# timmh/biolith

Hardware: AMD Instinct MI355X
Metric: effective samples/sec (psi) for occu NUTS, 10k sites x 5 visits (higher is better)
Workload: dtype f32; 1 GPU; biolith simulate(n_sites=10000, n_site_covs=3, n_obs_covs=3, 5 visits, seed 0); fit(occu): NUTS 4 chains per GPU x (1000 warmup + 1000 draws), one step = one full fit; chains_per_gpu=4, total_chains=4, num_warmup=1000, num_samples=1000, parallelism=chains x1 (1 process per GPU), wgs_per_chain=27, gather=none (one rank), env_overrides=

## Files before the change

### biolith_amd/csrc/biolith_hip.hip

```cpp
#include "../../include/biolith_hip.h"

#include <hip/hip_runtime.h>

#include <algorithm>
#include <cmath>
#include <cstdarg>
#include <cstdio>
#include <cstdlib>
#include <cstring>
#include <string>
#include <vector>

#include "logp_kernel.hpp"
#include "re_kernel.hpp"
#include "nuts_kernel.hpp"
#include "predict.hpp"
#include "site_posterior.hpp"
#include "abundance_posterior.hpp"
#include "path_posterior.hpp"
#include "score_posterior.hpp"
#include "count_posterior.hpp"
#include "comb_predict.hpp"
#include "predictive_check.hpp"
#include "predictive_density.hpp"
// ... 1700 lines not shown
        if (const char *e = bl_env(BL_ENV_RE_WGS)) k = atoi(e);
    }
    int ncu = 256;
    { hipDeviceProp_t prop; if (hipGetDeviceProperties(&prop, ds->device) == hipSuccess && prop.multiProcessorCount > 0) ncu = prop.multiProcessorCount; }
    k = std::max(1, std::min(std::min(k, 32), std::min(ncu * 7 / 8 / C, N * g.n_species)));
    const int nsp = g.n_species;
    int kps = std::max(1, k / nsp);
    const int nloc = (N + kps - 1) / kps;
    kps = (N + nloc - 1) / nloc;
    k = nsp * kps;
    if (k > 32) return bl_fail(BL_ERR_UNSUPPORTED, "n_species=%d needs %d workgroups per chain (at most 32)", nsp, k);
    if (C * k > ncu) return bl_fail(BL_ERR_UNSUPPORTED, "num_chains=%d random-effects chains need %d resident workgroups (%d CUs)", C, C * k, ncu);
    const int dl_max = g.G + nloc * per_site;

    const RunLayout RL = result_layout((size_t)C, Sa, D);
    size_t off = RL.end;
    auto carve = [&](size_t bytes) { size_t o = off; off = align256(off + bytes); return o; };
    const size_t o_draws = RL.draws, o_div = RL.div, o_steps = RL.steps, o_acc = RL.acc, o_pot = RL.pot, o_eps = RL.eps,
                 o_minv = RL.minv, o_nleap = RL.nleap, o_status = carve(16),
                 o_rng = carve((size_t)C * k * (dl_max + 2) * 16), o_init = carve((size_t)C * D * 4), o_dbg = carve(BL_DBG_SLOTS * 8),
                 o_xchg = carve((size_t)C * 2 * k * BL_RE_NRED_MAX * 8), o_loc = carve((size_t)C * 4), o_run = carve(sizeof(BlReRun));
    if (off > ds->run_bytes) {
        if (ds->d_run) hipFree(ds->d_run);
        ds->d_run = nullptr; ds->run_bytes = 0;
        BL_HIP(hipMalloc(&ds->d_run, off));
        ds->run_bytes = off;
    }
    const size_t state_bytes = (size_t)C * k * RE_SLOTS * dl_max * 4;
    if (state_bytes > ds->restate_bytes) {
        if (ds->d_restate) hipFree(ds->d_restate);
        ds->d_restate = nullptr; ds->restate_bytes = 0;
        BL_HIP(hipMalloc((void **)&ds->d_restate, state_bytes));
        ds->restate_bytes = state_bytes;
    }
    char *base = (char *)ds->d_run;
    ds->d_draws = (float *)(base + o_draws); ds->d_div = (unsigned char *)(base + o_div); ds->d_steps = (int *)(base + o_steps);
    ds->d_acc = (float *)(base + o_acc); ds->d_pot = (float *)(base + o_pot); ds->d_eps = (float *)(base + o_eps);
    ds->d_minv = (float *)(base + o_minv); ds->d_nleap = (long long *)(base + o_nleap); ds->d_status = (int *)(base + o_status);
    ds->d_rng = (uint32_t *)(base + o_rng); ds->d_init = (float *)(base + o_init); ds->d_dbg = (long long *)(base + o_dbg);
    ds->d_loc = (int *)(base + o_loc);

    const bool small_layout = D + 2 <= (size_t)BL_RNG_STREAMS_PER_CHAIN - 1;
    const int stride = small_layout ? BL_RNG_STREAMS_PER_CHAIN : (int)D + 2;
    const int ext_scalar = small_layout ? BL_RNG_STREAMS_PER_CHAIN - 1 : (int)D, ext_dir = small_layout ? BL_RNG_STREAMS_PER_CHAIN - 2 : (int)D + 1;
    std::vector<uint32_t> all((size_t)C * stride * 4), rs((size_t)C * k * (dl_max + 2) * 4, 0u);
    rng_streams_strided(cfg->seed, cfg->chain_offset, stride, C, all.data());
    for (int c = 0; c < C; c++)
        for (int w = 0; w < k; w++) {
            const int sp = w / kps, s0 = (w - sp * kps) * nloc, cnt = std::min(nloc, N - s0);
            uint32_t *dst = rs.data() + ((size_t)c * k + w) * (dl_max + 2) * 4;
            const uint32_t *src = all.data() + (size_t)c * stride * 4;
            auto put = [&](int local, int ext) { memcpy(dst + (size_t)local * 4, src + (size_t)ext * 4, 16); };
            int at = 0;
            for (; at < g.G; at++) put(at, at);
            if (g.site_re) {
                for (int i = 0; i < cnt; i++) put(at + i, g.o_u + sp * N + s0 + i);
                for (int i = 0; i < cnt; i++) put(at + cnt + i, g.o_v + sp * N + s0 + i);
                at += 2 * cnt;
            }
            if (g.obs_re)
                for (int v = 0; v < V; v++)
                    for (int i = 0; i < cnt; i++) put(at + v * cnt + i, g.o_e + (sp * N + s0 + i) * V + v);
            put(dl_max, ext_scalar);
            put(dl_max + 1, ext_dir);
        }
    BL_HIP(hipMemcpyAsync(ds->d_rng, rs.data(), rs.size() * 4, hipMemcpyHostToDevice, st));
    std::vector<float> it32;
    if (cfg->init_theta) {
        it32.resize((size_t)C * D);
        for (size_t i = 0; i < it32.size(); i++) it32[i] = (float)cfg->init_theta[i];
        BL_HIP(hipMemcpyAsync(ds->d_init, it32.data(), it32.size() * 4, hipMemcpyHostToDevice, st));
    }
    BlReRun run{};
    run.m = g;
    run.comb = ds->comb;
    const size_t lds = re_geometry(run.m, nloc, 1, dl_max);
    const bool cap4 = g.Ks <= 4 && g.Ko <= 4;
    run.num_chains = C; run.num_warmup = W; run.num_samples = S; run.max_depth = max_depth;
    run.k = k; run.nloc = nloc; run.dl_max = dl_max;
    run.xchg = (unsigned long long *)(base + o_xchg);
    { const char *e1 = bl_env(BL_ENV_NO_LOCAL); run.allow_local = (e1 && e1[0] == '1') ? 0 : 1; }
    run.xcd_local = ds->d_loc;
    run.target_accept = (float)(cfg->target_accept > 0.0 ? cfg->target_accept : 0.8);
    int32_t ws[32], we[32];
    run.nwin = adaptation_schedule(W, ws, we, 32);
    if (run.nwin > 32) return bl_fail(BL_ERR_INVALID, "adaptation schedule too long");
    for (int i = 0; i < 32; i++) run.win_end[i] = i < run.nwin ? we[i] : 0x7fffffff;
    run.state = ds->d_restate; run.rng = ds->d_rng;
    run.init_theta = cfg->init_theta ? ds->d_init : nullptr;
    run.abort_flag = ds->d_abort;
    run.draws = ds->d_draws; run.diverging = ds->d_div; run.num_steps = ds->d_steps; run.accept_prob = ds->d_acc;
    run.potential = ds->d_pot; run.step_size = ds->d_eps; run.inv_mass = ds->d_minv; run.nleap = ds->d_nleap; run.status = ds->d_status;
    run.dbg = ds->d_dbg;
    BlReRun *d_runp = (BlReRun *)(base + o_run);
    BL_HIP(hipMemcpyAsync(d_runp, &run, sizeof run, hipMemcpyHostToDevice, st));
    BL_HIP(hipStreamSynchronize(st));
    *ds->h_abort = 0;
    BL_HIP(hipEventRecord(ds->ev0, st));
    BL_HIP(hipMemsetAsync(ds->d_status, 0, 16, st));
    BL_HIP(hipMemsetAsync(ds->d_dbg, 0, BL_DBG_SLOTS * 8, st));
    BL_HIP(hipMemsetAsync(run.xchg, 0, (size_t)C * 2 * k * BL_RE_NRED_MAX * 8, st));
    BL_HIP(hipMemsetAsync(ds->d_loc, 0, (size_t)C * 4, st));
    BL_HIP(re_nuts_dispatch(cap4 ? 4 : 16, run, 8 * k * ((C + 7) / 8), lds, st));
    snprintf(ds->kernel_name, sizeof ds->kernel_name, "%s", g_kernel_name);
    BL_HIP(hipEventRecord(ds->ev1, st));
    ds->stream = st; ds->in_flight = true; ds->have_run = true;
    ds->C = C; ds->S = S; ds->W = W; ds->k = k; ds->nloc = nloc; ds->lds_ld = 0; ds->lds_bytes = (int)lds; ds->staged = run.m.lds_rows | (run.m.lds_hot << 1); ds->nvp = 0; ds->ncw = BL_RE_NW; ds->lane_grp = 0;
    return BL_OK;
}

extern "C" int bl_nuts_launch(bl_dataset *ds, const bl_nuts_config *cfg, void *stream)
{
    if (!ds || !cfg) return bl_fail(BL_ERR_INVALID, "NULL argument");
    if (ds->in_flight) return bl_fail(BL_ERR_BUSY, "a NUTS launch is already in flight on this handle");
    bl_env_snapshot();
    snprintf(ds->env_overrides, sizeof ds->env_overrides, "%s", bl_env_active().c_str());
    const int C = cfg->num_chains, S = cfg->num_samples, W = cfg->num_warmup, D = ds->D;
    if (C <= 0 || S < 0 || W < 0 || S + W <= 0) return bl_fail(BL_ERR_INVALID, "num_chains/num_samples/num_warmup out of range");
    if (C > 256) return bl_fail(BL_ERR_UNSUPPORTED, "num_chains=%d > 256 per device launch", C);
    const int max_depth = cfg->max_tree_depth > 0 ? cfg->max_tree_depth : 10;
    if (max_depth > BL_MAX_DEPTH) return bl_fail(BL_ERR_INVALID, "max_tree_depth > %d", BL_MAX_DEPTH);
    if (cfg->chain_offset < 0) return bl_fail(BL_ERR_INVALID, "chain_offset < 0");
    int rc = set_device(ds);
    if (rc) return rc;

    if (ds->model == 6) return re_nuts_launch(ds, cfg, (hipStream_t)stream, max_depth);

    int k, nloc, ld, lds_bytes, staged;
    int ncw, wide, grp;
    choose_geometry(ds, C, cfg->wgs_per_chain, &k, &nloc, &ld, &lds_bytes, &staged, &ncw, &wide, &grp);
    const int nvp = (D + 4 <= 16) ? 16 : (D + 4 <= 32 ? 32 : 64);

    const size_t Sa = S > 0 ? S : 1;
    const RunLayout RL = result_layout((size_t)C, Sa, (size_t)D);
    size_t off = RL.end;
    auto carve = [&](size_t bytes) { size_t o = off; off = align256(off + bytes); return o; };
    const size_t o_draws = RL.draws, o_div = RL.div, o_steps = RL.steps, o_acc = RL.acc, o_pot = RL.pot, o_eps = RL.eps,
                 o_minv = RL.minv, o_nleap = RL.nleap, o_status = carve(16),
                 o_rng = carve((size_t)C * BL_RNG_STREAMS_PER_CHAIN * 16), o_init = carve((size_t)C * D * 4), o_dbg = carve(BL_DBG_SLOTS * 8), o_loc = carve((size_t)C * 4),
                 o_cold = carve(sizeof(BlNutsCold));
    if (off > ds->run_bytes) {
        if (ds->d_run) hipFree(ds->d_run);
        ds->d_run = nullptr; ds->run_bytes = 0;
        BL_HIP(hipMalloc(&ds->d_run, off));
        ds->run_bytes = off;
    }
    char *base = (char *)ds->d_run;
    ds->d_draws = (float *)(base + o_draws); ds->d_div = (unsigned char *)(base + o_div); ds->d_steps = (int *)(base + o_steps);
    ds->d_acc = (float *)(base + o_acc); ds->d_pot = (float *)(base + o_pot); ds->d_eps = (float *)(base + o_eps);
    ds->d_minv = (float *)(base + o_minv); ds->d_nleap = (long long *)(base + o_nleap); ds->d_status = (int *)(base + o_status);
    ds->d_rng = (uint32_t *)(base + o_rng); ds->d_init = (float *)(base + o_init); ds->d_dbg = (long long *)(base + o_dbg); ds->d_loc = (int *)(base + o_loc);
    int pitch = nvp;
    { const char *e = bl_env(BL_ENV_PITCH); if (e && atoi(e) >= nvp && atoi(e) <= 4096) pitch = atoi(e); }
    const size_t xb = align256((size_t)C * BL_XCHG_SLOTS * k * pitch * 8);
    if (xb > ds->xchg_bytes) {
        if (ds->d_xchg) hipFree(ds->d_xchg);
        ds->d_xchg = nullptr; ds->xchg_bytes = 0;
        BL_HIP(hipMalloc((void **)&ds->d_xchg, xb));
        ds->xchg_bytes = xb;
    }

    hipStream_t st = (hipStream_t)stream;
    std::vector<uint32_t> rs((size_t)C * BL_RNG_STREAMS_PER_CHAIN * 4);
    for (int c = 0; c < C; c++)
        rng_streams(cfg->seed, cfg->chain_offset + c, BL_RNG_STREAMS_PER_CHAIN, rs.data() + (size_t)c * BL_RNG_STREAMS_PER_CHAIN * 4);
    BL_HIP(hipMemcpyAsync(ds->d_rng, rs.data(), rs.size() * 4, hipMemcpyHostToDevice, st));
    if (cfg->init_theta) {
        std::vector<float> it32((size_t)C * D);
        for (size_t i = 0; i < it32.size(); i++) it32[i] = (float)cfg->init_theta[i];
        BL_HIP(hipMemcpyAsync(ds->d_init, it32.data(), it32.size() * 4, hipMemcpyHostToDevice, st));
    }
    BlNutsCold cold{};
    cold.num_warmup = W; cold.num_samples = S;
    cold.target_accept = (float)(cfg->target_accept > 0.0 ? cfg->target_accept : 0.8);
    int32_t ws[32], we[32];
    cold.nwin = adaptation_schedule(W, ws, we, 32);
    if (cold.nwin > 32) return bl_fail(BL_ERR_INVALID, "adaptation schedule too long");
    for (int i = 0; i < 32; i++) cold.win_end[i] = i < cold.nwin ? we[i] : 0x7fffffff;
    cold.loc_b = ds->dd.loc_b; cold.isc2_b = ds->dd.isc2_b; cold.loc_a = ds->dd.loc_a; cold.isc2_a = ds->dd.isc2_a;
    cold.l1_b = ds->dd.l1_b; cold.l1_a = ds->dd.l1_a;
    cold.prior_const = ds->dd.prior_const;
    cold.fp_a = (float)ds->fp_a; cold.fp_b = (float)ds->fp_b;
    cold.rng = ds->d_rng;
    cold.init_theta = cfg->init_theta ? ds->d_init : nullptr;
    cold.abort_flag = ds->d_abort;
    cold.draws = ds->d_draws; cold.diverging = ds->d_div; cold.num_steps = ds->d_steps; cold.accept_prob = ds->d_acc;
    cold.potential = ds->d_pot; cold.step_size = ds->d_eps; cold.inv_mass = ds->d_minv; cold.nleap = ds->d_nleap;
    cold.status = ds->d_status; cold.xcd_local = ds->d_loc; cold.dbg = ds->d_dbg;
    BlNutsCold *d_cold = (BlNutsCold *)(base + o_cold);
    BL_HIP(hipMemcpyAsync(d_cold, &cold, sizeof cold, hipMemcpyHostToDevice, st));
    BL_HIP(hipStreamSynchronize(st));
    *ds->h_abort = 0;

    BlNutsParams p{};
    p.rows = ds->dd.rows; p.n_sites = ds->dd.n_sites; p.n_stride = ds->dd.n_stride;
    p.T = ds->dd.T; p.J = ds->dd.J; p.Ks = ds->dd.Ks; p.Ko = ds->dd.Ko;
    p.num_chains = C;
    p.k = k; p.nloc = nloc; p.rec_stride = ld; p.nvp = nvp;
    p.max_depth = max_depth;
    p.max_abundance = ds->max_abundance;
    p.rn_off = BL_OFF_DATA + ((nloc + 1) / 2) * ld * 4;
    p.lane_grp = ds->model == 8 ? dyn_lanes_per_pair(ds, C) : grp;
    p.nmix_lds = nmix_table_in_lds(ds, staged, nloc, &lds_bytes);
    p.grp_kernel = ((ds->model == 0 || ds->model == 2) && staged && (grp > 0 || ncw == BL_CWAVES_SINGLE)) ? 1 : 0;
    if (ncw == BL_CWAVES_SINGLE && k != 1) return bl_fail(BL_ERR_INVALID, "internal: %d compute waves are the one-workgroup form, k = %d", ncw, k);
    if (const char *e = bl_env(BL_ENV_GRP_KERNEL)) { if (e[0] == '1' && (ds->model == 0 || ds->model == 2) && staged) p.grp_kernel = 1; }
    p.fp_mode = ds->fp_mode;
    p.nmix_tab = ds->d_tab;
    p.ncw = ncw;
    p.n_species = ds->nsp; p.sp_lds = ((nloc + 1) / 2) * ld;
    if (ds->nsp > 1 && !staged)
        return bl_fail(BL_ERR_UNSUPPORTED, "joint sampling of %d species: the dataset slice does not fit the LDS-staged path", ds->nsp);
    p.wide = wide;
    p.xchg = ds->d_xchg;
    p.cold = d_cold;
    p.spin_limit = 5000000u;
    { const char *e = bl_env(BL_ENV_SPIN_US); if (e && atoi(e) > 0) p.spin_limit = (unsigned)atoi(e); }
    {
        const char *e1 = bl_env(BL_ENV_NO_LOCAL), *e2 = bl_env(BL_ENV_POLL_SLEEP);
        p.allow_local = (e1 && e1[0] == '1') ? 0 : 1;
        p.poll_sleep = e2 ? atoi(e2) : 3;
        if (p.poll_sleep < 0 || p.poll_sleep > 127) p.poll_sleep = 3;
        const char *e3 = bl_env(BL_ENV_FIRST_DELAY);
        p.pitch = pitch;
        p.first_delay = e3 ? atoi(e3) : 0;
        if (p.first_delay < 0 || p.first_delay > 127) p.first_delay = 0;
    }

    BL_HIP(hipEventRecord(ds->ev0, st));
    BL_HIP(hipMemsetAsync(ds->d_xchg, 0, xb, st));
    BL_HIP(hipMemsetAsync(ds->d_status, 0, 16, st));
    BL_HIP(hipMemsetAsync(ds->d_dbg, 0, BL_DBG_SLOTS * 8, st));
    BL_HIP(hipMemsetAsync(ds->d_loc, 0, (size_t)C * 4, st));
    const int grid = wide ? C * k : 8 * k * ((C + 7) / 8);
    if (ds->model != 0 && !staged)
        return bl_fail(BL_ERR_UNSUPPORTED, "occu_rn / false-positive model: the dataset slice does not fit the LDS-staged path");
    const int lrc = ds->kern->nuts(&p, grid, lds_bytes, staged, ds->model, st);
    if (lrc != 0) return bl_fail(BL_ERR_NO_DEVICE, "NUTS kernel launch failed: %s", hipGetErrorString((hipError_t)lrc));
    snprintf(ds->kernel_name, sizeof ds->kernel_name, "%s", g_kernel_name);
    BL_HIP(hipEventRecord(ds->ev1, st));
    ds->stream = st; ds->in_flight = true; ds->have_run = true;
    ds->C = C; ds->S = S; ds->W = W; ds->k = k; ds->nloc = nloc; ds->lds_ld = ld; ds->lds_bytes = lds_bytes; ds->staged = staged; ds->nvp = nvp; ds->ncw = ncw; ds->lane_grp = p.lane_grp;
    return BL_OK;
}

extern "C" int bl_nuts_poll(bl_dataset *ds, int *done)
{
    if (!ds || !done) return bl_fail(BL_ERR_INVALID, "NULL argument");
    if (!ds->in_flight) { *done = 1; return BL_OK; }
    hipSetDevice(ds->device);
    hipError_t e = hipEventQuery(ds->ev1);
    if (e == hipSuccess) { *done = 1; return BL_OK; }
    if (e == hipErrorNotReady) {
        (void)hipGetLastError();
        *done = 0;
        return BL_OK;
    }
    return bl_fail(BL_ERR_NO_DEVICE, "hipEventQuery: %s", hipGetErrorString(e));
}

extern "C" int bl_nuts_abort(bl_dataset *ds)
{
    if (!ds) return bl_fail(BL_ERR_INVALID, "NULL argument");
    if (ds->h_abort) __atomic_store_n(ds->h_abort, 1, __ATOMIC_SEQ_CST);
    return BL_OK;
}

extern "C" int bl_nuts_wait(bl_dataset *ds)
{
    if (!ds) return bl_fail(BL_ERR_INVALID, "NULL argument");
    if (!ds->have_run) return bl_fail(BL_ERR_INVALID, "no NUTS launch on this handle");
    int rc = set_device(ds);
    if (rc) return rc;
    if (ds->in_flight) {
        BL_HIP(hipEventSynchronize(ds->ev1));
        ds->in_flight = false;
    }
    int status = 0;
    BL_HIP(hipMemcpy(&status, ds->d_status, 4, hipMemcpyDeviceToHost));
    if (status == BL_ERR_TIMEOUT) return bl_fail(BL_ERR_TIMEOUT, "in-kernel exchange spin bound hit (a workgroup was not resident?)");
    if (status == BL_ERR_ABORTED) return bl_fail(BL_ERR_ABORTED, "sampling aborted on request");
    if (status != 0) return bl_fail(BL_ERR_NO_DEVICE, "kernel reported status %d", status);
    return BL_OK;
}

extern "C" int bl_nuts_fetch(bl_dataset *ds, bl_nuts_output *out)
{
    if (!ds || !out) return bl_fail(BL_ERR_INVALID, "NULL argument");
    if (!ds->have_run || ds->in_flight) return bl_fail(BL_ERR_BUSY, "no finished NUTS launch to fetch");
    int rc = set_device(ds);
    if (rc) return rc;
    const size_t C = ds->C, S = ds->S, D = ds->D;
    if (out->draws && S) BL_HIP(hipMemcpy(out->draws, ds->d_draws, C * S * D * 4, hipMemcpyDeviceToHost));
    if (out->diverging && S) BL_HIP(hipMemcpy(out->diverging, ds->d_div, C * S, hipMemcpyDeviceToHost));
    if (out->num_steps && S) BL_HIP(hipMemcpy(out->num_steps, ds->d_steps, C * S * 4, hipMemcpyDeviceToHost));
    if (out->accept_prob && S) BL_HIP(hipMemcpy(out->accept_prob, ds->d_acc, C * S * 4, hipMemcpyDeviceToHost));
    if (out->potential_energy && S) BL_HIP(hipMemcpy(out->potential_energy, ds->d_pot, C * S * 4, hipMemcpyDeviceToHost));
    if (out->step_size) BL_HIP(hipMemcpy(out->step_size, ds->d_eps, C * 4, hipMemcpyDeviceToHost));
    if (out->inv_mass) BL_HIP(hipMemcpy(out->inv_mass, ds->d_minv, C * D * 4, hipMemcpyDeviceToHost));
    if (out->n_leapfrog) BL_HIP(hipMemcpy(out->n_leapfrog, ds->d_nleap, C * 16, hipMemcpyDeviceToHost));
    return BL_OK;
}

extern "C" int bl_nuts_run(bl_dataset *ds, const bl_nuts_config *cfg, bl_nuts_output *out)
{
    int rc = bl_nuts_launch(ds, cfg, nullptr);
// ... 117 lines not shown
```

### biolith_amd/csrc/nuts_kernel.hpp

```cpp
#pragma once
#include "occu_device.hpp"

#ifdef BL_STAMPS
#define BL_STAMP_DECL long long st_acc[8] = {0, 0, 0, 0, 0, 0, 0, 0}; long long st_prev = (long long)clock64(); long long st_rt0 = (long long)wall_clock64(); long long st_spins = 0; \
    long long st_kn[3] = {0, 0, 0}, st_kc[3] = {0, 0, 0}; int st_kind = 0; long long st_sub[6] = {0, 0, 0, 0, 0, 0}; long long st_t = 0;
#define BL_STAMP(i) { const long long st_now = (long long)clock64(); st_acc[i] += st_now - st_prev; st_prev = st_now; }
#define BL_STAMP_KIND(k) st_kind = (k);
#define BL_STAMP_CRIT { const long long st_now = (long long)clock64(); st_kn[st_kind]++; st_kc[st_kind] += st_now - st_prev; }
#define BL_COUNT_SPINS(n) st_spins += (long long)(n);
#define BL_SUB0 st_t = (long long)clock64();
#define BL_SUB(i) { const long long st_n2 = (long long)clock64(); st_sub[i] += st_n2 - st_t; st_t = st_n2; }
#else
#define BL_SUB0
#define BL_SUB(i)
#define BL_COUNT_SPINS(n)
#define BL_STAMP_DECL
#define BL_STAMP(i)
#define BL_STAMP_KIND(k)
#define BL_STAMP_CRIT
#endif

struct BlNutsCold {
    int num_warmup, num_samples, nwin;
    float target_accept;
    int win_end[32];
    float loc_b, isc2_b, loc_a, isc2_a;
    float l1_b, l1_a;
    double prior_const;
    float fp_a, fp_b;
    const uint32_t *rng;
    const float *init_theta;
    const int *abort_flag;
    float *draws;
    unsigned char *diverging;
    int *num_steps;
    float *accept_prob;
    float *potential;
    float *step_size;
    float *inv_mass;
    long long *nleap;
    int *status;
    int *xcd_local;
    long long *dbg;
};
#define BL_DBG_SLOTS 544

struct BlNutsParams {
    const float *rows;
    int n_sites, n_stride, T, J, Ks, Ko;
    int num_chains;
    int k;
    int nloc;
    int rec_stride;
    int nvp;
    int ncw;
    int grp_kernel;
    int wide;
    const float *nmix_tab;
    int fp_mode;
    int max_depth;
    int max_abundance;
    int rn_off;
    int nmix_lds;
    int lane_grp;
    int allow_local;
    int poll_sleep;
    int first_delay;
    int pitch;
    int n_species;
    int sp_lds;
    unsigned spin_limit;
    unsigned long long *xchg;
    const BlNutsCold *cold;
};

struct BlCtlScalars {
    double U, Up;
    float wt, sumacc, eps;
    float da_xt, da_xavg, da_gavg, da_prox;
    int nprop, diverged, da_t, wf_n, win_idx, it;
    long long nleap_w, nleap_s;
};
enum { SV_TH = 0, SV_GR, SV_ZL, SV_RL, SV_GL, SV_ZR, SV_RR, SV_GRR, SV_ZP, SV_GP, SV_RSUM, SV_WFMEAN, SV_WFM2, SV_MOMZ };

__device__ __forceinline__ float bl_exp(float x) { return __builtin_amdgcn_exp2f(x * BL_LOG2E); }
__device__ __forceinline__ float bl_log(float x) { return BL_LN2 * __builtin_amdgcn_logf(x); }
__device__ __forceinline__ float bl_rcp(float x) { return __builtin_amdgcn_rcpf(x); }

__device__ __forceinline__ float bl_logaddexp(float a, float b)
{
    const float m = fmaxf(a, b);
    if (m == -INFINITY) return m;
    return m + bl_log(1.0f + bl_exp(-fabsf(a - b)));
}
__device__ __forceinline__ void bl_merge_weights(float a, float b, float &lse, float &pb)
{
    const float m = fmaxf(a, b);
    if (m == -INFINITY) { lse = m; pb = 0.0f; return; }
    const float d = b - a;
    const float e = bl_exp(-fabsf(d)), op = 1.0f + e;
    lse = m + bl_log(op);
    pb = (d > 0.0f ? 1.0f : e) * bl_rcp(op);
}

__device__ __forceinline__ bool bl_is_turning(float minv, float rl, float rr, float rsum, int D)
{
    const float rho = rsum - 0.5f * (rl + rr);
    float dl = minv * rl * rho, dr = minv * rr * rho;
    if (D <= 0) bl_low_sum2_w8(dl, dr); else bl_low_sum2(dl, dr, D);
    return (dl <= 0.0f) || (dr <= 0.0f);
}

__device__ __forceinline__ float bl_leaf_momentum(float rh, float epsdir, float g) { return fmaf(-0.5f * epsdir, g, rh); }
__device__ __forceinline__ void bl_next_leaf(float z, float r, float g, float epsdir, float minv, float &rh_out, float &z_out)
{
    const float rh = fmaf(-0.5f * epsdir, g, r);
    rh_out = rh;
    z_out = fmaf(epsdir * minv, rh, z);
}

__device__ __forceinline__ unsigned bl_xcc_id()
{
    unsigned x;
    asm volatile("s_getreg_b32 %0, hwreg(HW_REG_XCC_ID)" : "=s"(x));
    return x & 0xFu;
}

__device__ __forceinline__ unsigned long long bl_poll_load(const unsigned char *base, unsigned off)
{
    return __hip_atomic_load(reinterpret_cast<const unsigned long long *>(base + off), __ATOMIC_RELAXED, __HIP_MEMORY_SCOPE_AGENT);
}


struct BlSpinBound {
    unsigned spins = 0;
    long long deadline = 0;
    __device__ __forceinline__ bool expired(unsigned limit_us)
    {
        if ((++spins & 255u) != 0u) return false;
        const long long now = (long long)wall_clock64();
        if (deadline == 0) { deadline = now + (long long)limit_us * 100; return false; }
        return now > deadline;
    }
};

#define BL_XCHG_SLOTS 4u
#ifndef BL_COMPUTE_PRIO
#define BL_COMPUTE_PRIO 3
#endif
#ifndef BL_POLL_NB
#define BL_POLL_NB 2
#endif
#ifndef BL_RESIDENT_REC
#define BL_RESIDENT_REC 1
#endif
#ifndef BL_RESIDENT_MAX_FLOATS
#define BL_RESIDENT_MAX_FLOATS 96
#endif
#define SMALL_D_NVP(LEAN, MODEL, KS, KO) ((LEAN) && ((MODEL) == 0 || (MODEL) == 1) && (KS) + (KO) + 2 <= 8)
#ifndef BL_GRP_FORM
#define BL_GRP_FORM 2
#endif
template <int KS, int KO, bool LDS, int MODEL, int CW, bool GRP = false, int JSEL = -1, bool LEAN = false>
__global__ void __launch_bounds__(64 * (CW + 1)) bl_nuts_kernel(const BlNutsParams p)
{
    constexpr bool multi_wg = !(GRP && CW == BL_CWAVES_SINGLE);
    const int label = blockIdx.x & 7, slot = blockIdx.x >> 3;
    const int chain = p.wide ? (int)blockIdx.x / p.k : label + 8 * (slot / p.k);
    const int member = p.wide ? (int)blockIdx.x % p.k : slot % p.k;
    if (chain >= p.num_chains) return;
    const int tid = threadIdx.x, wave = tid >> 6, lane = tid & 63;
    const int Ks = p.Ks, Ko = p.Ko, nsp = (LEAN || (MODEL != 0 && MODEL != 2)) ? 1 : p.n_species;
    const int Dsp = Ks + Ko + 2;
    const int D = bl_model_dim<MODEL>(Ks, Ko, p.fp_mode) + (nsp - 1) * Dsp;
    constexpr bool ONE1 = LEAN && !GRP && MODEL == 0;
    const int T = ONE1 ? 1 : p.T, J = p.J;
    constexpr bool RESIDENT = BL_RESIDENT_REC && ONE1 && LDS && JSEL > 0 && BlPairRec<KS, KO, (JSEL > 0 ? JSEL : 1)>::FLOATS <= BL_RESIDENT_MAX_FLOATS;
    const int s0 = member * p.nloc;
    int cnt = p.n_sites - s0;
    cnt = cnt < 0 ? 0 : (cnt > p.nloc ? p.nloc : cnt);
    const float *grows = nullptr;
    int ld = p.rec_stride;
    if constexpr (MODEL == 1) {
        bl_rn_split_init<KS, KO, CW>(p.rows, p.n_stride, s0, cnt, T, J, p.rn_off);
        __syncthreads();
    }
    if constexpr (LDS) {
        for (int sp = 0; sp < nsp; sp++)
            bl_stage_records(p.rows, p.n_stride, s0, cnt, T, J, KS, bl_layout_ko<MODEL>(KO), p.rec_stride, 64 * (CW + 1), sp, sp * p.sp_lds, MODEL == 1 ? bl_rn_order<CW>(p.rn_off, cnt) : nullptr);
    } else {
        grows = p.rows + s0;
        ld = p.n_stride;
    }
    if constexpr (MODEL == 1) bl_rn_fill_lgamma(p.rn_off, p.max_abundance, 64 * (CW + 1));
    if constexpr (MODEL == 4) {
        if (p.nmix_lds) bl_stage_nmix_tab(p.nmix_tab + s0, p.n_stride, cnt, 2 * ((p.nloc + 1) / 2), T * (p.max_abundance + 1), p.rn_off, 64 * (CW + 1));
    }
    float *sh_coef = bl_lds_f(BL_OFF_COEF);
    int *sh_flag = bl_lds_i(BL_OFF_FLAG);
    float *sh_ckr = bl_lds_f(BL_OFF_CKR), *sh_ckrs = bl_lds_f(BL_OFF_CKRS);
    float *sv = bl_lds_f(BL_OFF_SV) + lane;
    BlCtlScalars *ss = reinterpret_cast<BlCtlScalars *>(bl_smem_raw + BL_OFF_SS);
    if (tid < 64) sh_coef[tid] = 0.0f;
    __syncthreads();

    const BlNutsCold *cold = p.cold;
    const bool act = lane < D;
    const bool is_phi = (MODEL == 2 || (MODEL == 3 && p.fp_mode != 0)) && lane == D - 1;
    const int lsp = lane < nsp * Dsp ? lane / Dsp : 0, lj = lane - lsp * Dsp;
    int my_pos = lane < nsp * Dsp ? lsp * BL_SP_COEF(KS, KO) + bl_coef_pos(lj, Ks, Ko, KS, KO) : nsp * BL_SP_COEF(KS, KO) + 1;
    int part_pos = lane < nsp * Dsp ? lsp * BL_SP_PART(KS, KO) + bl_coef_pos(lj, Ks, Ko, KS, KO) : (is_phi ? KS + KO + 3 : KS + KO + 2);
    bool beta_lane = lj <= Ks;
    if constexpr (MODEL == 8) {
        my_pos = part_pos = bl_dyn_pos(lane < D ? lane : D, Ks, Ko, KS, KO);
        beta_lane = lane < 3 * (Ks + 1);
    }
    const bool part_all = MODEL != 8 && lane >= nsp * Dsp;
    const int part_rs = nsp > 1 ? nsp * BL_SP_PART(KS, KO) : BL_PART_STRIDE;
    BlRng rng_d, rng_u, rng_dir;
    float minv = act ? 1.0f : 0.0f;
    float eps = 1.0f, epsdir = 0.f;
    double E0 = 0.0;
    int depth = 0;
    double sUp = 0.0;
    float szp = 0, sgp = 0, srsum = 0, swt = 0, ssumacc = 0;
    int snprop = 0;
    bool sdiv = false, sturn = false, going_right = false;
    float cz = 0, rh = 0;
    bool pend = false, pend_first = false, pend_end = false, pend_sturn = false, pend_sdiv = false;
    float pend_dE = 0.f, pend_z = 0.f, pend_g = 0.f;
    double pend_U = 0.0;
    int pend_snprop = 0;
    bool init_pending = true;
    float mom_r0 = 0.f;
    double mom_kin = 0.0;
    int end_kind = 0;
    bool local = false;
    float prior_loc = 0.f, prior_isc2 = 0.f, prior_l1 = 0.f;
    double prior_const = 0.0;
    int S = 0, W = 0, total = 0, nwin = 0, win_end_cur = 0;
    float target_accept = 0.8f;

    const int nvp = SMALL_D_NVP(LEAN, MODEL, KS, KO) ? 16 : p.nvp, G = 64 / nvp;
    const int c_idx = lane & (nvp - 1), sub = lane / nvp;
    const unsigned rec_bytes = (unsigned)(p.k * p.pitch * 8);
    const unsigned char *xbase = reinterpret_cast<const unsigned char *>(p.xchg) + (size_t)chain * BL_XCHG_SLOTS * rec_bytes;
    unsigned poff[8];
    float pval[8];
#pragma unroll
    for (int q = 0; q < 8; q++) {
        const int w = q * G + sub;
        poff[q] = (unsigned)(((w < p.k ? w : p.k - 1) * p.pitch + c_idx) * 8);
        pval[q] = (w < p.k) ? 1.0f : 0.0f;
    }
    const int nq = (p.k + G - 1) / G;
    const bool one_batch = LEAN || p.k <= 8 * G;

    if (wave == 0) {
        S = cold->num_samples; W = cold->num_warmup; total = W + S;
        target_accept = cold->target_accept; nwin = cold->nwin; win_end_cur = cold->win_end[0];
        prior_loc = beta_lane ? cold->loc_b : cold->loc_a;
        prior_isc2 = act ? (beta_lane ? cold->isc2_b : cold->isc2_a) : 0.0f;
        prior_l1 = act ? (beta_lane ? cold->l1_b : cold->l1_a) : 0.0f;
        if (is_phi) { prior_loc = cold->fp_a; prior_isc2 = cold->fp_b; prior_l1 = 0.0f; }
        prior_const = cold->prior_const;
        const uint32_t *rs = cold->rng + ((size_t)chain * BL_NSTREAM + lane) * 4;
        rng_d.s0 = rs[0]; rng_d.s1 = rs[1]; rng_d.s2 = rs[2]; rng_d.s3 = rs[3];
        const uint32_t *ru = cold->rng + ((size_t)chain * BL_NSTREAM + BL_SCALAR_STREAM) * 4;
        rng_u.s0 = ru[0]; rng_u.s1 = ru[1]; rng_u.s2 = ru[2]; rng_u.s3 = ru[3];
        const uint32_t *rd = cold->rng + ((size_t)chain * BL_NSTREAM + BL_DIR_STREAM) * 4;
        rng_dir.s0 = rd[0]; rng_dir.s1 = rd[1]; rng_dir.s2 = rd[2]; rng_dir.s3 = rd[3];
        const float u0 = bl_rng_uniform(rng_d);
        const float *init = cold->init_theta;
        cz = act ? (init ? init[chain * D + lane] : 4.0f * u0 - 2.0f) : 0.0f;
        if (act) sh_coef[my_pos] = cz;
        const float z_first = bl_rng_normal(rng_d);
        mom_r0 = act ? z_first : 0.0f;
        mom_kin = (double)(0.5f * bl_wave_sum(mom_r0 * mom_r0));
#pragma unroll
        for (int s = 0; s < 16; s++) sv[s * 64] = 0.0f;
        sv[SV_MOMZ * 64] = z_first;
        if (lane == 0) {
            sh_flag[0] = 0; sh_flag[1] = 0; sh_flag[2] = 0;
            for (int w = 0; w < 16; w++) bl_lds_i(BL_OFF_TAG)[w] = 0;
            BlCtlScalars z{};
            z.eps = 1.0f; z.da_prox = 2.302585093f;
            *ss = z;
        }
    }
    __syncthreads();

    constexpr bool SMALL_D = SMALL_D_NVP(LEAN, MODEL, KS, KO);
    const int Dred = (SMALL_D || D <= 8) ? 0 : D;
    float ck_last = 0.f, cks_last = 0.f;
    float t_zl = 0.f, t_rl = 0.f, t_gl = 0.f, t_zr = 0.f, t_rr = 0.f, t_gr = 0.f, t_rsum = 0.f, t_zp = 0.f, t_gp = 0.f;
    float t_wt = 0.f, t_sumacc = 0.f;
    double t_Up = 0.0;
    int t_nprop = 0, t_it = 0;
    auto mom_refresh = [&]() {
        mom_r0 = act ? sv[SV_MOMZ * 64] * __builtin_amdgcn_rsqf(minv) : 0.0f;
        mom_kin = (double)(0.5f * bl_wave_sum(minv * mom_r0 * mom_r0));
    };
    auto end_deferred = [&]() {
        if (end_kind == 0) return;
        const float th = t_zp, gr = t_gp, r0 = mom_r0;
        const double U = t_Up;
        const int nprop = t_nprop, it = t_it;
        if (end_kind & 2) {
            ss->nleap_w += nprop;
            if (end_kind & 4) {
                const int wf_n = ss->wf_n + 1;
                const float wf_mean0 = sv[SV_WFMEAN * 64];
                const float dpre = th - wf_mean0;
                const float wf_mean = wf_mean0 + dpre * bl_rcp((float)wf_n);
                sv[SV_WFMEAN * 64] = wf_mean;
                sv[SV_WFM2 * 64] += dpre * (th - wf_mean);
                ss->wf_n = wf_n;
            }
            if (end_kind & 8) {
                const int wi = ss->win_idx + 1;
                ss->win_idx = wi;
                win_end_cur = cold->win_end[wi < 31 ? wi : 31];
            }
        } else if (end_kind & 16) {
            ss->nleap_s += nprop;
            if (member == 0) {
                const size_t s = (size_t)chain * S + (it - W);
                if (act) cold->draws[s * D + lane] = th;
                if (lane == 0) {
                    cold->num_steps[s] = nprop;
                    cold->accept_prob[s] = t_sumacc * bl_rcp((float)nprop);
                    cold->diverging[s] = pend_sdiv ? 1 : 0;
                    cold->potential[s] = (float)U;
                }
            }
        }
        if (end_kind & (2 | 16)) t_it = it + 1;
        end_kind = 0;
        t_zl = th; t_rl = r0; t_gl = gr;
        t_zr = th; t_rr = r0; t_gr = gr;
        t_rsum = r0;
        t_wt = 0.f; t_sumacc = 0.f; t_nprop = 0;
        const float z = bl_rng_normal(rng_d);
        sv[SV_MOMZ * 64] = z;
        mom_r0 = act ? z * __builtin_amdgcn_rsqf(minv) : 0.0f;
        mom_kin = (double)(0.5f * bl_wave_sum(minv * mom_r0 * mom_r0));
    };

    auto run_deferred = [&]() {
        if (!pend) return;
        pend = false;
        const float lw = -pend_dE;
        const float lacc = pend_dE <= 0.0f ? 1.0f : bl_exp(-pend_dE);
        if (pend_first) {
            szp = pend_z; sgp = pend_g; sUp = pend_U; swt = lw; ssumacc = lacc;
        } else {
            float pr, lse;
            bl_merge_weights(swt, lw, lse, pr);
            const float u = bl_rng_uniform(rng_u);
            if (u < pr) { szp = pend_z; sgp = pend_g; sUp = pend_U; }
            swt = lse;
            ssumacc += lacc;
        }
        if (pend_end) {
            const float wt = t_wt;
            float pr = fminf(1.0f, bl_exp(swt - wt));
            if (pend_sturn || pend_sdiv) pr = 0.0f;
            const float u = bl_rng_uniform(rng_u);
            if (u < pr) { t_zp = szp; t_gp = sgp; t_Up = sUp; }
            t_wt = bl_logaddexp(wt, swt);
            t_sumacc += ssumacc;
            t_nprop += pend_snprop;
        }
    };

    unsigned epoch = 0;
    bool have_pending = false, p_timed_out = false;
    double p_acc = 0.0;
    float p_cg = 0.f, p_pe2 = 0.f;
    float cz_spec = 0.f;
    int flag = 0;
    BL_STAMP_DECL
    constexpr bool SPEC = LDS && MODEL != 1;
#ifndef BL_RN_HYBRID
#define BL_RN_HYBRID 2
#endif
    constexpr bool HYBRID = BL_RN_HYBRID && LDS && MODEL == 1;
    auto decide = [&]() {
        have_pending = false;
        const double acc = p_acc;
        const float cg = p_cg, pe2 = p_pe2;
        const double ll_tot = bl_readlane_d(acc, D);
        const bool abort_req = bl_readlane_d(acc, D + 1) != 0.0;
        flag = 0;
        if (p_timed_out) flag = 4;
        else if (abort_req) flag = 5;
        bool new_transition = false;
        BL_STAMP_KIND(0)
        if (flag == 0) {
            if (init_pending) {
                BL_STAMP_KIND(2)
                BL_SUB0
                const double Un = -ll_tot + (double)(0.5f * bl_wave_sum(pe2)) + prior_const;
                init_pending = false;
                new_transition = true;
                t_zp = cz; t_gp = cg; t_Up = Un;
                end_kind = 1;
            } else {
                const float cr = bl_leaf_momentum(rh, epsdir, cg);
                float s_prior = pe2, s_kin = minv * cr * cr;
                if (SMALL_D || Dred <= 0) bl_low_sum2_w8(s_prior, s_kin); else bl_low_sum2(s_prior, s_kin, D);
                const double Un = -ll_tot + (double)(0.5f * s_prior) + prior_const;
                const double Kn = (double)(0.5f * s_kin);
                double dE = (Un + Kn) - E0;
                if (dE != dE) dE = (double)INFINITY;
                const int leaf_idx = snprop;
                sdiv = dE > 1000.0;
                srsum = (leaf_idx == 0) ? cr : srsum + cr;
                snprop = leaf_idx + 1;
                pend = true; pend_first = (leaf_idx == 0); pend_end = false;
                pend_dE = (float)dE; pend_U = Un; pend_z = cz; pend_g = cg;
                const int idx_max = __popc((unsigned)leaf_idx >> 1);
                const int idx_min = idx_max - (int)__builtin_ctz(~(unsigned)leaf_idx) + 1;
                if ((leaf_idx & 1) == 0) {
                    sh_ckr[idx_max * 64 + lane] = cr;
                    sh_ckrs[idx_max * 64 + lane] = srsum;
                    ck_last = cr; cks_last = srsum;
                } else {
                    sturn = bl_is_turning(minv, ck_last, cr, srsum - cks_last + ck_last, SMALL_D ? 0 : Dred);
                    for (int i = idx_max - 1; i >= idx_min && !sturn; i--) {
                        const float ck = sh_ckr[i * 64 + lane];
                        const float srs = srsum - sh_ckrs[i * 64 + lane] + ck;
                        sturn = bl_is_turning(minv, ck, cr, srs, SMALL_D ? 0 : Dred);
                    }
                }
                if (snprop < (1 << depth) && !sturn && !sdiv) {
                    bl_next_leaf(cz, cr, cg, epsdir, minv, rh, cz);
                } else {
                    BL_STAMP_KIND(1)
                    pend_end = true; pend_sturn = sturn; pend_sdiv = sdiv; pend_snprop = snprop;
                    const float o_z = going_right ? t_zl : t_zr, r_other = going_right ? t_rl : t_rr, o_g = going_right ? t_gl : t_gr;
                    if (going_right) { t_zr = cz; t_rr = cr; t_gr = cg; } else { t_zl = cz; t_rl = cr; t_gl = cg; }
                    const float rsum = t_rsum + srsum;
                    t_rsum = rsum;
                    const bool turning = sturn || bl_is_turning(minv, going_right ? r_other : cr, going_right ? cr : r_other, rsum, Dred);
                    depth++;
                    if (depth < p.max_depth && !turning && !sdiv) {
                        const bool was_right = going_right;
                        going_right = (bl_rng_next(rng_dir) >> 31) != 0u;
                        epsdir = going_right ? eps : -eps;
                        snprop = 0; sturn = false; sdiv = false;
                        float ez = cz, er = cr, eg = cg;
                        if (going_right != was_right) { ez = o_z; er = r_other; eg = o_g; }
                        bl_next_leaf(ez, er, eg, epsdir, minv, rh, cz);
                    } else {
                        BL_STAMP_KIND(2)
                        BL_SUB0
                        run_deferred();
                        BL_SUB(0)
                        const int it = t_it;
                        end_kind = it < W ? (1 | 2) : (1 | 16);
                        if (it < W) {
                            const float accp = t_sumacc * bl_rcp((float)t_nprop);
                            const float g = target_accept - accp;
                            const int da_t = ss->da_t + 1;
                            const float tt = (float)da_t;
                            const float rt10 = bl_rcp(tt + 10.0f);
                            const float da_gavg = (1.0f - rt10) * ss->da_gavg + g * rt10;
                            const float da_xt = ss->da_prox - __builtin_amdgcn_sqrtf(tt) * 20.0f * da_gavg;
                            const float wgt = __builtin_amdgcn_exp2f(-0.75f * __builtin_amdgcn_logf(tt));
                            const float da_xavg = (1.0f - wgt) * ss->da_xavg + wgt * da_xt;
                            eps = bl_exp((it == W - 1) ? da_xavg : da_xt);
                            eps = fminf(fmaxf(eps, 1.1754944e-38f), 3.4028235e+38f);
                            ss->da_t = da_t; ss->da_gavg = da_gavg; ss->da_xt = da_xt; ss->da_xavg = da_xavg;
                            const int win_idx = ss->win_idx;
                            const bool middle = win_idx > 0 && win_idx < nwin - 1;
                            const bool at_end = it == win_end_cur;
                            if (middle) end_kind |= 4;
                            if (at_end) end_kind |= 8;
                            if (at_end && middle) {
                                const float th = t_zp;
                                const int wf_n = ss->wf_n + 1;
                                const float wf_mean0 = sv[SV_WFMEAN * 64];
                                const float dpre = th - wf_mean0;
                                const float wf_mean = wf_mean0 + dpre * bl_rcp((float)wf_n);
                                const float wf_m2 = sv[SV_WFM2 * 64] + dpre * (th - wf_mean);
                                const float n = (float)wf_n;
                                const float var = wf_m2 * bl_rcp(n - 1.0f), rn5 = bl_rcp(n + 5.0f);
                                minv = act ? (n * rn5 * var + 1e-3f * 5.0f * rn5) : 0.0f;
                                sv[SV_WFMEAN * 64] = 0.f; sv[SV_WFM2 * 64] = 0.f; ss->wf_n = 0;
                                end_kind &= ~4;
                                ss->da_xt = 0.f; ss->da_xavg = 0.f; ss->da_gavg = 0.f; ss->da_t = 0;
                                ss->da_prox = bl_log(10.0f * eps);
                                mom_refresh();
                            }
                        }
                        if (it + 1 >= total) flag = 1;
                        else new_transition = true;
                        BL_SUB(1)
                    }
                }
            }
            if (new_transition) {
                const float th = t_zp, gr = t_gp;
                const float r0 = mom_r0;
                E0 = t_Up + mom_kin;
                depth = 0;
                going_right = (bl_rng_next(rng_dir) >> 31) != 0u;
                epsdir = going_right ? eps : -eps;
                snprop = 0; sturn = false; sdiv = false;
                bl_next_leaf(th, r0, gr, epsdir, minv, rh, cz);
                BL_SUB(2)
            }
        }
        if (flag != 0) end_deferred();
        if (flag != 0 && member == 0) {
            if (flag > 1 && lane == 0) atomicMax(cold->status, flag);
            if (act) cold->inv_mass[chain * D + lane] = minv;
            if (lane == 0) {
                cold->step_size[chain] = eps;
                cold->nleap[chain * 2 + 0] = ss->nleap_w;
                cold->nleap[chain * 2 + 1] = ss->nleap_s;
                cold->xcd_local[chain] = local ? 1 : 0;
            }
        }
    };

    if (wave > 0) {
        if constexpr (BL_COMPUTE_PRIO > 0 && MODEL != 1 && multi_wg) __builtin_amdgcn_s_setprio(BL_COMPUTE_PRIO);
        unsigned epoch_c = 0;
        const int lane_grp = MODEL == 1 ? bl_rn_npos(p.rn_off) : p.lane_grp;
        BlPairRec<KS, KO, (RESIDENT ? JSEL : 1)> rrec;
        bool rvalid = false;
        float rvmask = 0.0f;
        if constexpr (RESIDENT) bl_load_resident_rec(tid - 64, ld, cnt, rrec, rvalid, rvmask);
        while (true) {
            typedef int BlInt2 __attribute__((ext_vector_type(2)));
            const BlInt2 ctl = *(__attribute__((address_space(3))) const volatile BlInt2 *)sh_flag;
#ifdef BL_STAMPS
            const long long st_a0 = (long long)clock64();
#endif
            if constexpr (RESIDENT) bl_phase_a_rec(wave - 1, rrec, rvalid, rvmask);
            else bl_phase_a<KS, KO, LDS, MODEL, CW, GRP ? BL_GRP_FORM : 0, JSEL, ONE1>(tid - 64, wave - 1, grows, ld, cnt, T, J, p.max_abundance, p.fp_mode, p.nmix_tab + s0, (MODEL == 4 && p.nmix_lds) ? 2 * ((p.nloc + 1) / 2) : p.n_stride, nsp, p.sp_lds, p.rn_off, lane_grp, p.nmix_lds);
#ifdef BL_STAMPS
            st_sub[5] += (long long)clock64() - st_a0; st_sub[4]++;
#endif
            if (ctl.x != 0) break;
            const bool local_c = ctl.y != 0;
            epoch_c++;
            if (multi_wg) {
            typedef __attribute__((address_space(3))) volatile unsigned BlLdsU;
            typedef __attribute__((address_space(3))) const volatile float BlLdsF;
            BlLdsU *tags = (BlLdsU *)bl_lds_i(BL_OFF_TAG);
            BlLdsF *part = (BlLdsF *)(bl_lds_f(BL_OFF_PART) + part_pos);
            asm volatile("" ::: "memory");
            if (lane == 0) tags[wave - 1] = epoch_c;
            unsigned stale = 0u;
#pragma unroll
            for (int w = 0; w < CW; w++) stale |= tags[w] ^ epoch_c;
            float row[CW];
#pragma unroll
            for (int w = 0; w < CW; w++) row[w] = part[w * part_rs];
            if (__builtin_amdgcn_readfirstlane(stale) == 0u) {
                float comp = row[0];
#pragma unroll
                for (int w = 1; w < CW; w++) comp += row[w];
                for (int sp = 1; sp < nsp; sp++) {
#pragma unroll
                    for (int w = 0; w < CW; w++) comp += part_all ? (float)part[w * part_rs + sp * BL_SP_PART(KS, KO)] : 0.0f;
                }
                if (lane > D) comp = 0.0f;
                if (lane == D + 1 && member == 0 && (epoch_c & 255u) == 0u)
                    comp = (__hip_atomic_load(cold->abort_flag, __ATOMIC_RELAXED, __HIP_MEMORY_SCOPE_SYSTEM) != 0) ? 1.0f : 0.0f;
                if (epoch_c == 1u) {
                    const float xcc = (float)bl_xcc_id();
                    if (lane == D + 2) comp = xcc;
                    if (lane == D + 3) comp = xcc * xcc;
                }
                const unsigned char *rbase = xbase + (epoch_c & (BL_XCHG_SLOTS - 1u)) * rec_bytes;
                const unsigned long long granule = ((unsigned long long)epoch_c << 32) | __float_as_uint(comp);
                if (lane < nvp) {
                    int lane_o = lane;
                    asm volatile("" : "+v"(lane_o));
                    const unsigned store_off = (unsigned)((member * p.pitch + (lane_o & (nvp - 1))) * 8);
                    unsigned long long *dst = reinterpret_cast<unsigned long long *>(const_cast<unsigned char *>(rbase) + store_off);
                    if (local_c)
                        __hip_atomic_store(dst, granule, __ATOMIC_RELAXED, __HIP_MEMORY_SCOPE_WORKGROUP);
                    else
                        __hip_atomic_store(dst, granule, __ATOMIC_RELAXED, __HIP_MEMORY_SCOPE_AGENT);
                }
            }
            }
            __syncthreads();
            __syncthreads();
        }
    } else {
    int run_status = 0;
    while (true) {
        bool redo = false;
        if ((SPEC || HYBRID) && have_pending) {
            end_deferred();
            decide();
            redo = flag != 0 || __any(act && !(cz == cz_spec));
            if (flag == 0) run_deferred();
            BL_STAMP_CRIT
            BL_STAMP(0)
        } else if (!SPEC) {
            end_deferred();
            run_deferred();
            BL_STAMP(0)
        } else {
            end_deferred();
            BL_STAMP(0)
        }
        float pe2 = 0.0f, pg = 0.0f;
        int spec_kind = 0;
        float spec_ed = epsdir, spec_other = 0.0f;
        if (!redo) {
        const float dth = cz - prior_loc;
        pe2 = fmaf(dth * dth, prior_isc2, 2.0f * fabsf(dth) * prior_l1);
        pg = fmaf(dth, prior_isc2, dth > 0.0f ? prior_l1 : (dth < 0.0f ? -prior_l1 : 0.0f));
        if constexpr (MODEL == 2) {
            if (is_phi) {
                const float e = bl_exp(-fabsf(cz)), op = 1.0f + e, l = bl_log(op);
                const float sig = (cz > 0.0f ? 1.0f : e) * bl_rcp(op);
                pe2 = 2.0f * (prior_loc * (fmaxf(-cz, 0.0f) + l) + prior_isc2 * (fmaxf(cz, 0.0f) + l));
                pg = (prior_loc + prior_isc2) * sig - prior_loc;
            }
        }
        if constexpr (MODEL == 3) {
            if (is_phi) {
                const float rf = prior_loc * bl_exp(fminf(cz, 80.0f));
                pe2 = 2.0f * (rf - cz);
                pg = rf - 1.0f;
            }
        }
        spec_ed = epsdir;
        if constexpr (HYBRID) {
            if (!init_pending && ((snprop & 1) == 0 || BL_RN_HYBRID == 2) && snprop + 1 < (1 << depth)) spec_kind = 1;
        }
        if constexpr (SPEC) {
            if (!init_pending) {
                if (snprop + 1 < (1 << depth)) spec_kind = 1;
                else if (depth + 1 < p.max_depth) {
                    BlRng peek = rng_dir;
                    const bool gr2 = (bl_rng_next(peek) >> 31) != 0u;
                    spec_ed = gr2 ? eps : -eps;
                    spec_kind = 2;
                    if (gr2 != going_right) {
                        float rh2;
                        bl_next_leaf(gr2 ? t_zr : t_zl, gr2 ? t_rr : t_rl, gr2 ? t_gr : t_gl, spec_ed, minv, rh2, spec_other);
                        spec_kind = 3;
                    }
                }
            }
        }
        }
        __syncthreads();
        BL_STAMP(1)

        epoch++;
        if (redo) {
            if (act) sh_coef[my_pos] = cz;
            if (lane == 0) sh_flag[0] = flag;
            run_status = flag;
        } else {
            const unsigned char *rbase = xbase + (epoch & (BL_XCHG_SLOTS - 1u)) * rec_bytes;
            BL_STAMP(2)
            for (int z = 0; z < p.first_delay; z++) __builtin_amdgcn_s_sleep(1);
            double acc = 0.0;
            bool timed_out = false;
            if (!multi_wg) {
                const float *part = bl_lds_f(BL_OFF_PART) + part_pos;
                float comp = part[0];
#pragma unroll
                for (int w = 1; w < CW; w++) comp += part[w * part_rs];
                for (int sp = 1; sp < nsp; sp++) {
#pragma unroll
                    for (int w = 0; w < CW; w++) comp += part_all ? part[w * part_rs + sp * BL_SP_PART(KS, KO)] : 0.0f;
                }
                if (lane > D) comp = 0.0f;
                if (lane == D + 1 && (epoch & 255u) == 0u)
                    comp = (__hip_atomic_load(cold->abort_flag, __ATOMIC_RELAXED, __HIP_MEMORY_SCOPE_SYSTEM) != 0) ? 1.0f : 0.0f;
                acc = (double)comp;
            } else if (one_batch) {
                unsigned long long v[8];
                BlSpinBound bound;
                while (true) {
#ifdef BL_STAMPS
                    const long long st_r0 = (long long)clock64();
#endif
#pragma unroll
                    for (int q = 0; q < 8; q += 2) {
                        if (q < nq) {
                            v[q] = bl_poll_load(rbase, poff[q]);
                            v[q + 1] = bl_poll_load(rbase, poff[q + 1]);
                        } else {
                            v[q] = v[0];
                            v[q + 1] = v[0];
                        }
                    }
                    unsigned bad = 0u;
#pragma unroll
                    for (int q = 0; q < 8; q++) bad |= ((unsigned)(v[q] >> 32)) ^ epoch;
                    const bool all_in = __all(bad == 0u);
#ifdef BL_STAMPS
                    st_sub[3] += (long long)clock64() - st_r0;
#endif
                    if (all_in) break;
                    if (bound.expired(p.spin_limit)) { timed_out = true; break; }
                    if (!local)
                        for (int z = 0; z < p.poll_sleep; z++) __builtin_amdgcn_s_sleep(1);
                }
                BL_COUNT_SPINS(bound.spins)
#pragma unroll
                for (int q = 0; q < 8; q++) acc += (double)(pval[q] * __uint_as_float((unsigned)v[q]));
            } else {
                constexpr int NB = MODEL == 1 ? 1 : BL_POLL_NB;
                for (int p0 = 0; p0 < p.k && !timed_out; p0 += NB * 8 * G) {
                    unsigned long long v[NB][8];
                    BlSpinBound bound;
                    while (true) {
                        unsigned bad = 0u;
#pragma unroll
                        for (int b = 0; b < NB; b++) {
                            if (b == 0 || p0 + b * 8 * G < p.k) {
#pragma unroll
                                for (int q = 0; q < 8; q++) {
                                    const int w = p0 + (b * 8 + q) * G + sub;
                                    v[b][q] = bl_poll_load(rbase, (unsigned)(((w < p.k ? w : p.k - 1) * p.pitch + c_idx) * 8));
                                }
                            } else {
#pragma unroll
                                for (int q = 0; q < 8; q++) v[b][q] = v[0][0];
                            }
                        }
#pragma unroll
                        for (int b = 0; b < NB; b++)
#pragma unroll
                            for (int q = 0; q < 8; q++) bad |= ((unsigned)(v[b][q] >> 32)) ^ epoch;
                        if (__all(bad == 0u)) break;
                        if (bound.expired(p.spin_limit)) { timed_out = true; break; }
                        if (!local)
                            for (int z = 0; z < p.poll_sleep; z++) __builtin_amdgcn_s_sleep(1);
                    }
#pragma unroll
                    for (int b = 0; b < NB; b++)
#pragma unroll
                        for (int q = 0; q < 8; q++) {
                            const int w = p0 + (b * 8 + q) * G + sub;
                            acc += (w < p.k) ? (double)__uint_as_float((unsigned)v[b][q]) : 0.0;
                        }
                }
            }
            if (multi_wg) {
                if (nvp <= 16) acc = bl_fold_rows16_d(acc);
                if (nvp <= 32) acc = bl_fold_halves32_d(acc);
            }
            BL_STAMP(3)
            if (epoch == 1u && p.allow_local) {
                const double sx = bl_readlane_d(acc, D + 2), sxx = bl_readlane_d(acc, D + 3);
                local = ((double)p.k * sxx == sx * sx);
                if (lane == 0) sh_flag[1] = local ? 1 : 0;
            }
            const float cg = act ? (-(float)acc + pg) : 0.0f;
            p_acc = acc; p_cg = cg; p_pe2 = pe2; p_timed_out = timed_out;
            have_pending = true;
            cz_spec = __builtin_nanf("");
            if (!SPEC && !(HYBRID && spec_kind != 0 && !timed_out)) {
                decide();
                if (act) sh_coef[my_pos] = cz;
                if (lane == 0) sh_flag[0] = flag;
                run_status = flag;
                BL_STAMP_CRIT
            } else {
            if (spec_kind != 0 && !timed_out) {
                if (spec_kind == 3) cz_spec = spec_other;
                else {
                    const float cr = bl_leaf_momentum(rh, epsdir, cg);
                    float rh2;
                    bl_next_leaf(cz, cr, cg, spec_ed, minv, rh2, cz_spec);
                }
            }
            if (act && cz_spec == cz_spec) sh_coef[my_pos] = cz_spec;
            if (lane == 0) sh_flag[0] = 0;
            run_status = 0;
            }
            BL_STAMP(4)
        }
        __syncthreads();
        BL_STAMP(5)
        if (run_status != 0) break;
    }
    }
#ifdef BL_STAMPS
    if (cold->dbg && chain == 0 && member == 0 && tid == 0) {
        for (int i = 0; i < 8; i++) cold->dbg[i] = st_acc[i];
        cold->dbg[8] = (long long)epoch;
        cold->dbg[9] = (long long)wall_clock64() - st_rt0;
        cold->dbg[10] = st_spins;
        for (int i = 0; i < 3; i++) { cold->dbg[11 + i] = st_kn[i]; }
        cold->dbg[14] = st_kc[0]; cold->dbg[15] = st_kc[1]; cold->dbg[7] = st_kc[2];
        for (int i = 0; i < 4; i++) cold->dbg[16 + i] = st_sub[i];
    }
    if (cold->dbg && chain == 0 && member < 32 && wave >= 1 && wave <= 8 && (tid & 63) == 0) {
        cold->dbg[32 + member * 8 + (wave - 1)] = st_sub[5];
        unsigned hw;
        asm volatile("s_getreg_b32 %0, hwreg(HW_REG_HW_ID)" : "=s"(hw));
        cold->dbg[32 + 256 + member * 8 + (wave - 1)] = (long long)hw;
    }
    if (cold->dbg && chain == 0 && member < 32 && wave == 0 && tid == 0) {
        unsigned hw;
        asm volatile("s_getreg_b32 %0, hwreg(HW_REG_HW_ID)" : "=s"(hw));
        cold->dbg[32 + 256 + member * 8 + 7] = (long long)hw;
    }
    if (cold->dbg && chain == 0 && member == 0 && tid == 64) {
        cold->dbg[20] = st_sub[4]; cold->dbg[21] = st_sub[5];
        if constexpr (MODEL == 1) for (int i = 0; i < 8; i++) cold->dbg[22 + i] = bl_rn_dbg[i];
    }
#endif
}
```

Measured before the change: 274,600 ESS/s.

## Poll exchange records as interleaved 128-bit granule pairs with permlane swap

Interleaves the exchange granules so each lane can poll two granules with one 128-bit buffer load. The partial sums are then redistributed with permlane32_swap and a DPP fold, replacing eight 64-bit polls per lane. Granule store positions and readlane indices are remapped to match the new layout, and the pitch is rounded up to even. This aims to cut memory transactions and latency in the cross-workgroup spin-wait on the critical path, at the cost of a more intricate lane mapping that applies only to small-D lean models.

```diff
diff --git a/biolith_amd/csrc/biolith_hip.hip b/biolith_amd/csrc/biolith_hip.hip
--- a/biolith_amd/csrc/biolith_hip.hip
+++ b/biolith_amd/csrc/biolith_hip.hip
@@ -1876,6 +1876,7 @@
     ds->d_rng = (uint32_t *)(base + o_rng); ds->d_init = (float *)(base + o_init); ds->d_dbg = (long long *)(base + o_dbg); ds->d_loc = (int *)(base + o_loc);
     int pitch = nvp;
     { const char *e = bl_env(BL_ENV_PITCH); if (e && atoi(e) >= nvp && atoi(e) <= 4096) pitch = atoi(e); }
+    pitch += pitch & 1;
     const size_t xb = align256((size_t)C * BL_XCHG_SLOTS * k * pitch * 8);
     if (xb > ds->xchg_bytes) {
         if (ds->d_xchg) hipFree(ds->d_xchg);
diff --git a/biolith_amd/csrc/nuts_kernel.hpp b/biolith_amd/csrc/nuts_kernel.hpp
--- a/biolith_amd/csrc/nuts_kernel.hpp
+++ b/biolith_amd/csrc/nuts_kernel.hpp
@@ -158,6 +158,12 @@
 #define BL_RESIDENT_MAX_FLOATS 96
 #endif
 #define SMALL_D_NVP(LEAN, MODEL, KS, KO) ((LEAN) && ((MODEL) == 0 || (MODEL) == 1) && (KS) + (KO) + 2 <= 8)
+#ifndef BL_POLL_PAIRS
+#define BL_POLL_PAIRS 1
+#endif
+__host__ __device__ __forceinline__ constexpr int bl_pair_pos(int v) { return v < 8 ? 2 * v : 2 * (v - 8) + 1; }
+__host__ __device__ __forceinline__ constexpr int bl_pair_lane(int v) { return v < 8 ? v : 24 + v; }
+typedef unsigned BlU4 __attribute__((ext_vector_type(4)));
 #ifndef BL_GRP_FORM
 #define BL_GRP_FORM 2
 #endif
@@ -255,6 +261,19 @@
     }
     const int nq = (p.k + G - 1) / G;
     const bool one_batch = LEAN || p.k <= 8 * G;
+    constexpr bool PAIRS = BL_POLL_PAIRS && SMALL_D_NVP(LEAN, MODEL, KS, KO) && multi_wg;
+    unsigned ppoff[4] = {0u, 0u, 0u, 0u};
+#define BL_XL(v) (PAIRS ? bl_pair_lane(v) : (v))
+    if constexpr (PAIRS) {
+        const int psub = (lane >> 3) & 3;
+#pragma unroll
+        for (int q = 0; q < 4; q++) {
+            const int w = 4 * (2 * q + (lane >> 5)) + psub;
+            ppoff[q] = (unsigned)(((w < p.k ? w : p.k - 1) * p.pitch + 2 * (lane & 7)) * 8);
+        }
+#pragma unroll
+        for (int q = 0; q < 8; q++) pval[q] = (4 * q + psub < p.k) ? 1.0f : 0.0f;
+    }
 
     if (wave == 0) {
         S = cold->num_samples; W = cold->num_warmup; total = W + S;
@@ -390,8 +409,8 @@
         have_pending = false;
         const double acc = p_acc;
         const float cg = p_cg, pe2 = p_pe2;
-        const double ll_tot = bl_readlane_d(acc, D);
-        const bool abort_req = bl_readlane_d(acc, D + 1) != 0.0;
+        const double ll_tot = bl_readlane_d(acc, BL_XL(D));
+        const bool abort_req = bl_readlane_d(acc, BL_XL(D + 1)) != 0.0;
         flag = 0;
         if (p_timed_out) flag = 4;
         else if (abort_req) flag = 5;
@@ -582,7 +601,8 @@
                 if (lane < nvp) {
                     int lane_o = lane;
                     asm volatile("" : "+v"(lane_o));
-                    const unsigned store_off = (unsigned)((member * p.pitch + (lane_o & (nvp - 1))) * 8);
+                    const int gran = lane_o & (nvp - 1);
+                    const unsigned store_off = (unsigned)((member * p.pitch + (PAIRS ? bl_pair_pos(gran) : gran)) * 8);
                     unsigned long long *dst = reinterpret_cast<unsigned long long *>(const_cast<unsigned char *>(rbase) + store_off);
                     if (local_c)
                         __hip_atomic_store(dst, granule, __ATOMIC_RELAXED, __HIP_MEMORY_SCOPE_WORKGROUP);
@@ -683,6 +703,41 @@
                 if (lane == D + 1 && (epoch & 255u) == 0u)
                     comp = (__hip_atomic_load(cold->abort_flag, __ATOMIC_RELAXED, __HIP_MEMORY_SCOPE_SYSTEM) != 0) ? 1.0f : 0.0f;
                 acc = (double)comp;
+            } else if (PAIRS) {
+                const int nqp = (nq + 1) >> 1;
+                const __amdgpu_buffer_rsrc_t rsrc = __builtin_amdgcn_make_buffer_rsrc(const_cast<unsigned char *>(xbase), (short)0, (int)(BL_XCHG_SLOTS * rec_bytes), 0x00020000);
+                const int soff = (int)((epoch & (BL_XCHG_SLOTS - 1u)) * rec_bytes);
+                BlU4 v[4];
+                BlSpinBound bound;
+                while (true) {
+#ifdef BL_STAMPS
+                    const long long st_r0 = (long long)clock64();
+#endif
+                    asm volatile("" ::: "memory");
+#pragma unroll
+                    for (int q = 0; q < 4; q++) {
+                        if (q < nqp) v[q] = __builtin_amdgcn_raw_buffer_load_b128(rsrc, (int)ppoff[q], soff, 16);
+                        else v[q] = BlU4{0u, epoch, 0u, epoch};
+                    }
+                    unsigned bad = 0u;
+#pragma unroll
+                    for (int q = 0; q < 4; q++) bad |= (v[q].y ^ epoch) | (v[q].w ^ epoch);
+                    const bool all_in = __all(bad == 0u);
+#ifdef BL_STAMPS
+                    st_sub[3] += (long long)clock64() - st_r0;
+#endif
+                    if (all_in) break;
+                    if (bound.expired(p.spin_limit)) { timed_out = true; break; }
+                    if (!local)
+                        for (int z = 0; z < p.poll_sleep; z++) __builtin_amdgcn_s_sleep(1);
+                }
+                BL_COUNT_SPINS(bound.spins)
+#pragma unroll
+                for (int q = 0; q < 4; q++) {
+                    const auto r = __builtin_amdgcn_permlane32_swap(v[q].x, v[q].z, false, false);
+                    acc += (double)(pval[2 * q] * __uint_as_float(r[0]));
+                    acc += (double)(pval[2 * q + 1] * __uint_as_float(r[1]));
+                }
             } else if (one_batch) {
                 unsigned long long v[8];
                 BlSpinBound bound;
@@ -753,13 +808,16 @@
                         }
                 }
             }
-            if (multi_wg) {
+            if (PAIRS) {
+                acc += bl_dpp_d<0x128, 0xF>(acc);
+                acc = bl_fold_rows16_d(acc);
+            } else if (multi_wg) {
                 if (nvp <= 16) acc = bl_fold_rows16_d(acc);
                 if (nvp <= 32) acc = bl_fold_halves32_d(acc);
             }
             BL_STAMP(3)
             if (epoch == 1u && p.allow_local) {
-                const double sx = bl_readlane_d(acc, D + 2), sxx = bl_readlane_d(acc, D + 3);
+                const double sx = bl_readlane_d(acc, BL_XL(D + 2)), sxx = bl_readlane_d(acc, BL_XL(D + 3));
                 local = ((double)p.k * sxx == sx * sx);
                 if (lane == 0) sh_flag[1] = local ? 1 : 0;
             }
```

Result: faster. 286,800 ESS/s (median of 6 runs) (+4.4%).
